# ectucker1/voxel-raytracing

Measured on AMD Instinct MI355X. Metric: Mrays/sec at 1080p treehouse.vox; achieved HBM GB/s vs MI355X peak, higher is better.
Workload: dtype f32; 1 GPU; synthetic:treehouse(seed=2) 256^3 stand-in for treehouse.vox, 1920x1080, primary rays only (BASELINE configs[1]); 128 frame(s)/step (128 per GPU, consecutive poses, one K1 launch per step), 16-row strips over 1 GPU(s); traversal=AUTO, bytes_out_per_px=37, device=AMD Radeon Graphics (gfx950:sramecc+:xnack-)

## Files before the change

voxel-raytracing_amd/csrc/vrt_api.hip:

```cpp
#include <cstdio>
#include <cstdlib>
#include <cstring>

#include "image_io.h"
#include "vox_reader.h"
#include "vrt_host.h"

using namespace vrt;

static thread_local std::string g_err;

int vrt::fail(int code, const std::string& msg) { g_err = msg; return code; }

struct OptName { const char* name; const char* env; int DevOptions::*field; };
static const OptName kOptNames[] = {
    {"tile_tags", "VRT_TILE_TAGS", &DevOptions::tile_tags}, {"box_rect", "VRT_BOX_RECT", &DevOptions::box_rect},
    {"xcd_regions", "VRT_XCD_REGIONS", &DevOptions::xcd_regions}, {"fast_loop", "VRT_FAST_LOOP", &DevOptions::fast_loop},
    {"no_bounce_kernel", "VRT_NO_BOUNCE_KERNEL", &DevOptions::no_bounce_kernel}, {"sky_fast", "VRT_SKY_FAST", &DevOptions::sky_fast},
    {"sky_span", "VRT_SKY_SPAN", &DevOptions::sky_span},
    {"packed_bounces", "VRT_PACKED_BOUNCES", &DevOptions::packed_bounces}, {"ao_batch", "VRT_AO_BATCH", &DevOptions::ao_batch}, {"tags_async", "VRT_TAGS_ASYNC", &DevOptions::tags_async},
    {"hit_table", "VRT_HIT_TABLE", &DevOptions::hit_table},
    {"thresh_runs", "VRT_THRESH_RUNS", &DevOptions::thresh_runs}, {"denoise_th16", "VRT_DENOISE_TH", &DevOptions::denoise_th16}, {"denoise_packed", "VRT_DENOISE_PACKED", &DevOptions::denoise_packed},
    {"denoise_pair", "VRT_DENOISE_PAIR", &DevOptions::denoise_pair}, {"denoise_p0", "VRT_DENOISE_P0", &DevOptions::denoise_p0}, {"denoise_pair_wgs", "VRT_DENOISE_PAIR_WGS", &DevOptions::denoise_pair_wgs},
    {"denoise_verified", "VRT_DENOISE_VERIFIED", &DevOptions::denoise_verified}, {"denoise_guard_div8", "VRT_DENOISE_GUARD_DIV8", &DevOptions::denoise_guard_div8},
    {"denoise_count", "VRT_DENOISE_COUNT", &DevOptions::denoise_count},
    {"open_cells", "VRT_OPEN_CELLS", &DevOptions::open_cells}, {"df_prefetch", "VRT_DF_PREFETCH", &DevOptions::df_prefetch},
    {"df_own", "VRT_DF_OWN", &DevOptions::df_own},
};

extern "C" {

const char* vrt_last_error(void) { return g_err.c_str(); }

int vrt_ctx_create(int device, vrt_ctx** out)
{
    if (!out) return fail(VRT_ERR_INVALID, "vrt_ctx_create: out is NULL");
    int n = 0;
    hipError_t e = hipGetDeviceCount(&n);
    if (e != hipSuccess || n <= 0)
        return fail(VRT_ERR_NO_DEVICE, std::string("no HIP device available (") + hipGetErrorString(e) +
                                           "); this library has no CPU fallback");
    if (device < 0 || device >= n) return fail(VRT_ERR_INVALID, "vrt_ctx_create: device index out of range");
    HIPCHK(hipSetDevice(device));
    vrt_ctx* c = new vrt_ctx();
    c->device = device;
    for (const OptName& o : kOptNames) {
        const char* e = getenv(o.env);
        if (e && e[0] >= '0' && e[0] <= '9') c->opt.*(o.field) = atoi(e);
    }
    if (hipStreamCreateWithFlags(&c->stream, hipStreamNonBlocking) != hipSuccess) { delete c; return fail(VRT_ERR_HIP, "hipStreamCreate failed"); }
    hipEventCreate(&c->ev_geo0); hipEventCreate(&c->ev_prim1); hipEventCreate(&c->ev_geo1);
    hipEventCreate(&c->ev_den0); hipEventCreate(&c->ev_den1);
    *out = c;
    return VRT_OK;
}

void vrt_ctx_destroy(vrt_ctx* c)
{
    if (!c) return;
    hipSetDevice(c->device);
    hipStreamSynchronize(c->stream);
    if (c->tag_stream) { hipStreamSynchronize(c->tag_stream); hipStreamDestroy(c->tag_stream); }
    for (int b = 0; b < 2; b++) {
        if (c->tag_done[b]) hipEventDestroy(c->tag_done[b]);
        if (c->tag_read[b]) hipEventDestroy(c->tag_read[b]);
    }
    if (c->upload_stream) { hipStreamSynchronize(c->upload_stream); hipStreamDestroy(c->upload_stream); }
    for (int i = 0; i < vrt_ctx::kTabRing; i++) {
        if (c->tab_host[i]) hipHostFree(c->tab_host[i]);
        if (c->tab_uploaded[i]) hipEventDestroy(c->tab_uploaded[i]);
        if (c->tab_consumed[i]) hipEventDestroy(c->tab_consumed[i]);
    }
// ... 341 lines not shown
    p.xcd_turn = (n > 1 && p.tiles_y_local > 0 && ceil_div(p.tiles_y_local, 8) * 8 * 100 > p.tiles_y_local * 103) ? 1 : 0;
    p.wgs_per_frame_rcp = p.wgs_per_frame ? (uint32_t)(0x100000000ull / (uint64_t)p.wgs_per_frame) : 0u;
    {
        const bool want = opt.xcd_regions != 0;
        if (want && n >= 8 && p.sh.nranks == 1 && p.tile_h == 8 && p.tiles_x >= 4 && p.tiles_y_local >= 8) {
            const uint32_t rw = ((uint32_t)p.tiles_x + 1u) / 2u, rh = ((uint32_t)p.tiles_y_local + 3u) / 4u;
            p.xcd_turn = 2;
            p.wgs_per_frame = rw * rh;
            p.wgs_per_frame_rcp = (uint32_t)(0x100000000ull / (uint64_t)p.wgs_per_frame);
            p.tiles_y_rcp = (uint32_t)(0x100000000ull / (uint64_t)rw);
        }
    }
    p.tps = (uint32_t)(p.sh.strip_rows / p.tile_h);
    p.tiles_x_rcp = (uint32_t)(0x100000000ull / (uint64_t)p.tiles_x);
    if (p.xcd_turn != 2) p.tiles_y_rcp = p.tiles_y_local ? (uint32_t)(0x100000000ull / (uint64_t)p.tiles_y_local) : 0u;
    p.tps_rcp = (uint32_t)(0x100000000ull / (uint64_t)p.tps);
    p.fused_shade = (st->ao_samples == 0 && st->shadows == 0 && (st->max_bounces == 0 || !s->metallic_voxels)) ? 1 : ((st->flags & VRT_FLAG_SPLIT_KERNELS) ? 0 : 2);
    p.no_bounce = ((st->max_bounces == 0 || !s->metallic_voxels) && opt.no_bounce_kernel) ? 1 : 0;
    p.sc.vol.ao_batch = (opt.ao_batch && p.sc.vol.df_own) ? 1u : 0u;
    p.packed_chain = (opt.packed_bounces && st->ao_samples <= 0xFFFFu && (!s->bricks || opt.packed_bounces >= 2)) ? 1 : 0;
    {
        const bool want = opt.fast_loop != 0;
        const bool df = st->traversal == VRT_TRAVERSAL_AUTO || st->traversal == VRT_TRAVERSAL_DF;
        const bool sec = p.fused_shade != 1;
        bool ok = want && df && s->d.vol.df_fast && st->max_steps >= 1 && st->max_steps <= 1024 && p.tile_h == 8 &&
                  !(st->flags & (VRT_FLAG_DEBUG_PLANES | 2u)) && (!sec || st->ao_samples == 0 || (st->ao_steps >= 1 && st->ao_steps <= 1024));
        for (int f = 0; f < n && ok; f++) ok = frames[f].hit_voxel == nullptr;
        p.fast_loop = ok ? ((counts || (st->flags & VRT_FLAG_MARCHED_COUNTS)) ? 2 : 1) : 0;
        if (s->bricks && (counts || (st->flags & (VRT_FLAG_MARCHED_COUNTS | VRT_FLAG_DEBUG_PLANES | 2u)))) p.fast_loop = 2;
        const int dmax = s->d.vol.W > s->d.vol.H ? (s->d.vol.W > s->d.vol.D ? s->d.vol.W : s->d.vol.D) : (s->d.vol.H > s->d.vol.D ? s->d.vol.H : s->d.vol.D);
        p.sc.vol.df_thresh = (ok && opt.thresh_runs && !counts && dmax <= 1022 && st->max_steps >= 32) ? 1u : 0u;
        if (s->bricks) p.sc.vol.df_thresh = (opt.thresh_runs && !counts && !(st->flags & (VRT_FLAG_DEBUG_PLANES | 2u)) && st->max_steps >= 32) ? 1u : 0u;
    }
    {
        bool ok = opt.sky_fast != 0 && s->d.skyk.w != 0u && !(st->flags & (VRT_FLAG_DEBUG_PLANES | 2u));
        for (int f = 0; f < n && ok; f++)
            ok = !frames[f].color_f && !frames[f].hit_voxel && !frames[f].hit_mask && !frames[f].steps_primary && !frames[f].steps_total && !frames[f].rays_total;
        p.sky_fast = ok ? 1 : 0;
    }
    p.occ2_bytes = s->occ2_bytes; p.occ3_bytes = s->occ3_bytes;
    p.occ_in_lds = ((size_t)s->occ2_bytes + s->occ3_bytes <= 65536) ? 1 : 0;
    {
        TileMap& m = p.map;
        bool six = p.sky_fast != 0;
        for (int f = 0; f < n && six; f++)
            six = frames[f].color8 && frames[f].depth && frames[f].motion && frames[f].mask8 && frames[f].position && frames[f].normal8 &&
                  !frames[f].hit_id && !frames[f].color8_strips;
        m.flags = (st->flags & 0xFFFFu) | (p.sky_fast ? VRT_MAPFLAG_SKY_FAST : 0u) | (six ? VRT_MAPFLAG_SIX : 0u) |
                  ((p.sky_fast && opt.sky_span) ? VRT_MAPFLAG_SKY_SPAN : 0u); m.n_frames = p.n_frames; m.xcd_turn = p.xcd_turn;
        m.wgs_per_frame = p.wgs_per_frame; m.wgs_per_frame_rcp = p.wgs_per_frame_rcp;
        m.tiles_x = p.tiles_x; m.tiles_x_rcp = p.tiles_x_rcp; m.tiles_y_local = p.tiles_y_local; m.tiles_y_rcp = p.tiles_y_rcp;
        m.tps = p.tps; m.tps_rcp = p.tps_rcp; m.tile = p.tile_h; m.nranks = p.sh.nranks; m.strip_rows = p.sh.strip_rows;
        m.W = p.W; m.H = p.H;
    }
    return VRT_OK;
}

static int launch_records(vrt_ctx* c, size_t px, GeomParams& p)
{
    if (c->records_px < px) {
        HIPCHK(hipStreamSynchronize(c->stream));
        c->records.reset(); c->hit_list.reset(); c->records_px = 0;
        HIPCHK(c->records.alloc(px * sizeof(uint4)));
        HIPCHK(c->hit_list.alloc((px + 1) * sizeof(uint32_t)));
        c->records_px = px;
    }
    p.records = c->records.get();
    p.hit_list = c->hit_list.get();
    p.hit_count = c->hit_list.get() + c->records_px;
    HIPCHK(hipMemsetAsync(p.hit_count, 0, sizeof(uint32_t), c->stream));
    return VRT_OK;
}

static int launch_tags(vrt_ctx* c, const vrt_scene* s, const Launch& l, const FrameSlot* slots, int tab, bool counts, GeomParams& p, int* tag_buf)
{
    const int n = l.n;
    bool want = c->opt.tile_tags != 0 && s->cells_ok && !counts && l.W <= 8128 && l.H <= 8128;
    bool any = false;
    for (int f = 0; f < n && want && !any; f++) any = !(slots[f].box[0] == 0 && slots[f].box[1] == 255 && slots[f].box[2] == 0 && slots[f].box[3] == 255);
    const bool tags = want && any;
    p.tags_x = tags ? (uint32_t)(p.tiles_x * (p.tile_w / 8)) : 0u; p.tags_y = tags ? (uint32_t)(p.tiles_y_local * (p.tile_h / 8)) : 0u;
    p.tags_per_frame = p.tags_x * p.tags_y + 1u;
    const size_t words = (size_t)p.tags_per_frame * (size_t)n;
    const int b = c->tag_flip; c->tag_flip ^= 1;
    *tag_buf = b;
    if (c->tile_tags_words[b] < words) {
        HIPCHK(hipStreamSynchronize(c->stream));
        if (c->tag_stream) HIPCHK(hipStreamSynchronize(c->tag_stream));
        c->tile_tags[b].reset(); c->tile_tags_words[b] = 0;
        HIPCHK(c->tile_tags[b].alloc(words * sizeof(uint32_t)));
        HIPCHK(hipMemsetAsync(c->tile_tags[b].get(), 0, words * sizeof(uint32_t), c->stream));
        HIPCHK(hipStreamSynchronize(c->stream));
        c->tile_tags_words[b] = words;
        c->tag_read_valid[b] = false;
    }
    if (++c->tile_gen == 0u) {
        HIPCHK(hipStreamSynchronize(c->stream));
        if (c->tag_stream) HIPCHK(hipStreamSynchronize(c->tag_stream));
        for (int q = 0; q < 2; q++)
            if (c->tile_tags[q]) HIPCHK(hipMemsetAsync(c->tile_tags[q].get(), 0, c->tile_tags_words[q] * sizeof(uint32_t), c->stream));
        HIPCHK(hipStreamSynchronize(c->stream));
        c->tile_gen = 1u;
    }
    p.tile_tags = c->tile_tags[b].get(); p.tile_gen = c->tile_gen;
    if (!tags) {
        std::vector<uint32_t> ones((size_t)n, c->tile_gen);
// ... 196 lines not shown
```

voxel-raytracing_amd/csrc/vrt_device.hip:

```cpp
#include "vrt_device_common.h"

namespace vrt {


struct RayHit {
    uint32_t material;
    f3 pos, normal, dir;
    uint32_t ncode;
};

typedef const __attribute__((address_space(3))) uint64_t* lds_u64_ptr;
template <bool LDS> struct OccT;
template <> struct OccT<true>  { lds_u64_ptr o2, o3; };
template <> struct OccT<false> { const uint64_t* o2; const uint64_t* o3; };

__device__ __forceinline__ f3 hit_normal(uint32_t mask, int sx, int sy, int sz)
{
    const uint32_t k = __builtin_popcount(mask & 7u);
    const float c = k == 1u ? 1.0f : (k == 2u ? __uint_as_float(0x3f3504f3u) : __uint_as_float(0x3f13cd3au));
    const bool general = ((mask & 1u) && sx == 0) || ((mask & 2u) && sy == 0) || ((mask & 4u) && sz == 0);
    f3 n = mk3((mask & 1u) ? (float)(-sx) : 0.0f, (mask & 2u) ? (float)(-sy) : 0.0f, (mask & 4u) ? (float)(-sz) : 0.0f);
    if (general) return normalize3(n);
    return mk3(n.x * c, n.y * c, n.z * c);
}
// ... 729 lines not shown
        }
    }
    if (MODE != 0) {
        f3 col;
        if (MODE >= 5) {
            PixCtx c; c.px = px; c.py = py; c.fetches = 0; c.rays = 0; c.pc = SlotOf<TABLE>::push(P, frame);
            c.ldsw = (uint32_t)(uintptr_t)(lds_u64_ptr)lds_occ + (uint32_t)wave * (uint32_t)VRT_AO_SLOT;
            f3 colh = mk3(0.0f, 0.0f, 0.0f);
            if (__ballot(hit) != 0ull) colh = color_main_ray_packed<TRAV, OccT<kLds>, (MODE == 5 ? 2 : (MODE == 6 ? 5 : VRT_MAX_BOUNCES))>(P, occ, c, h, hit);
            if (hit) {
                col = colh;
                if (VRT_COUNTS(TRAV) && steps_total && !(P.st.flags & 3u)) steps_total[i] = r.fetches + c.fetches;
                if (rays_total && !(P.st.flags & 3u)) rays_total[i] = 1u + c.rays;
            } else {
                col = sky_color(s, dir);
                if (VRT_COUNTS(TRAV) && steps_total && P.sc.vol.count_lookups != 0u && !(P.st.flags & 3u)) steps_total[i] = r.fetches + c.fetches;
            }
        } else if (hit) {
            PixCtx c; c.px = px; c.py = py; c.fetches = 0; c.rays = 0; c.pc = SlotOf<TABLE>::push(P, frame);
            c.ldsw = (uint32_t)(uintptr_t)(lds_u64_ptr)lds_occ + (uint32_t)wave * (uint32_t)VRT_AO_SLOT;
            if (MODE == 1) col = color_hit<TRAV, OccT<kLds>, false>(P, occ, c, h, mk3(0.0f, 0.0f, 0.0f), 0);
            else {
                col = color_main_ray<TRAV, OccT<kLds>, MODE != 4>(P, occ, c, h);
                if (VRT_COUNTS(TRAV) && steps_total && !(P.st.flags & 3u)) steps_total[i] = r.fetches + c.fetches;
                if (rays_total && !(P.st.flags & 3u)) rays_total[i] = 1u + c.rays;
            }
        } else {
            col = sky_color(s, dir);
        }
#ifdef VRT_EXP_LATE_INDEX
        {
            int pxl = px, pyl = py;
            asm volatile("" : "+v"(pxl), "+v"(pyl));
            const size_t il = (size_t)pyl * (size_t)W + (size_t)pxl;
            store_color(f, col, il, (uint32_t)il, ((uint32_t)(yp0 + (pyl - y0)) * (uint32_t)W + (uint32_t)pxl) << 2);
        }
#else
        store_color(f, col, i, i32, ((uint32_t)(yp0 + (py - y0)) * (uint32_t)W + (uint32_t)px) << 2);
#endif
#ifdef VRT_EXP_STAMPS
        if (f.motion) *gptr<vrt_f2>(f.motion, i32 << 3) = (vrt_f2){__uint_as_float((uint32_t)t_begin), __uint_as_float((uint32_t)wall_clock64())};
#endif
    } else if (hit) {
        uint32_t packed = h.material | (r.mask << 8) | ((uint32_t)(r.sx + 1) << 11) | ((uint32_t)(r.sy + 1) << 13) |
                          ((uint32_t)(r.sz + 1) << 15);
        P.records[i] = make_uint4(__float_as_uint(h.pos.x), __float_as_uint(h.pos.y), __float_as_uint(h.pos.z), packed);
        uint32_t slot = atomicAdd(P.hit_count, 1u);
        P.hit_list[slot] = (uint32_t)i;
    } else {
        store_color(f, sky_color(s, dir), i, i32, ((uint32_t)(yp0 + (py - y0)) * (uint32_t)W + (uint32_t)px) << 2);
    }
}


template <int TRAV, bool OCC_LDS>
__global__ __launch_bounds__(256) void k_shade(const GeomParams P)
{
    extern __shared__ __attribute__((aligned(16))) uint64_t lds_occ[];
    constexpr bool kLds = OCC_LDS && (TRAV == VRT_TRAVERSAL_BITMASK || TRAV == VRT_TRAVERSAL_JUMP);
    uint32_t count = *P.hit_count;
    if (blockIdx.x * 256u >= count) return;
    const OccT<kLds> occ = stage_occ<kLds>(P, lds_occ);
    uint32_t gid = blockIdx.x * 256u + threadIdx.x;
    if (gid >= count) return;
    size_t i = P.hit_list[gid];
    int W = P.W;
    int px = (int)(i % (size_t)W), py = (int)(i / (size_t)W);

    uint4 rec = P.records[i];
    RayHit h;
    h.material = rec.w & 0xFFu;
    h.dir = primary_dir(P.slot[0], px, py);
    h.pos = mk3(__uint_as_float(rec.x), __uint_as_float(rec.y), __uint_as_float(rec.z));
    uint32_t mask = (rec.w >> 8) & 7u;
    int sx = (int)((rec.w >> 11) & 3u) - 1, sy = (int)((rec.w >> 13) & 3u) - 1, sz = (int)((rec.w >> 15) & 3u) - 1;
    PixCtx c; c.px = px; c.py = py; c.fetches = 0; c.rays = 0; c.pc = &P.slot[0].pc;
    c.ldsw = (uint32_t)(uintptr_t)(lds_u64_ptr)lds_occ + (uint32_t)__builtin_amdgcn_readfirstlane((int)(threadIdx.x >> 6)) * (uint32_t)VRT_AO_SLOT;
    h.normal = hit_normal(mask, sx, sy, sz);
    {
        const bool general = (mask & 7u) == 0u || ((mask & 1u) && sx == 0) || ((mask & 2u) && sy == 0) || ((mask & 4u) && sz == 0);
        h.ncode = general ? 0xFFFFFFFFu : ((mask & 7u) | ((uint32_t)(sx < 0) << 3) | ((uint32_t)(sy < 0) << 4) | ((uint32_t)(sz < 0) << 5));
    }
    f3 col = color_main_ray<TRAV>(P, occ, c, h);
    const vrt_frame& f = P.slot[0].fr;
    if (f.color_f) { f.color_f[i * 3 + 0] = col.x; f.color_f[i * 3 + 1] = col.y; f.color_f[i * 3 + 2] = col.z; }
    if (f.color8 || f.color8_strips) {
        uchar4 c8; c8.x = unorm8(col.x); c8.y = unorm8(col.y); c8.z = unorm8(col.z); c8.w = 0;
        if (f.color8) reinterpret_cast<uchar4*>(f.color8)[i] = c8;
        if (f.color8_strips) {
            int strip = py / P.sh.strip_rows;
            int yp = (strip / P.sh.nranks) * P.sh.strip_rows + (py - strip * P.sh.strip_rows);
            reinterpret_cast<uchar4*>(f.color8_strips)[(size_t)yp * (size_t)P.W + (size_t)px] = c8;
        }
    }
    if (VRT_COUNTS(TRAV) && f.steps_total) f.steps_total[i] += c.fetches;
    if (f.rays_total) f.rays_total[i] += c.rays;
}


template <int TRAV, bool OCC_LDS, int MODE, bool TABLE>
static void launch_k1_map(const GeomParams& p, dim3 grid, dim3 block, size_t lds, hipStream_t s)
{
    if constexpr (TRAV == VRT_TRAVERSAL_DF_FAST || TRAV == VRT_TRAVERSAL_BRICK) {
        if (p.xcd_turn == 0) { hipLaunchKernelGGL((k_primary<TRAV, OCC_LDS, MODE, TABLE, 0>), grid, block, lds, s, p); return; }
        if (p.xcd_turn == 2) { hipLaunchKernelGGL((k_primary<TRAV, OCC_LDS, MODE, TABLE, 2>), grid, block, lds, s, p); return; }
    }
    hipLaunchKernelGGL((k_primary<TRAV, OCC_LDS, MODE, TABLE, -1>), grid, block, lds, s, p);
}

template <int TRAV, bool OCC_LDS, bool TABLE>
static hipError_t launch_k1(const GeomParams& p, dim3 grid, dim3 block, size_t lds, hipStream_t s)
{
    constexpr bool kProduct = TRAV == VRT_TRAVERSAL_DF_FAST || TRAV == VRT_TRAVERSAL_DF_FAST_CNT || TRAV == VRT_TRAVERSAL_BRICK || TRAV == VRT_TRAVERSAL_BRICK_CNT;
    if (p.fused_shade == 1) launch_k1_map<TRAV, OCC_LDS, 1, TABLE>(p, grid, block, lds, s);
    else if (p.fused_shade == 2) {
        if (p.no_bounce) launch_k1_map<TRAV, OCC_LDS, 4, TABLE>(p, grid, block, lds, s);
        else if (kProduct && p.packed_chain) {
            if constexpr (kProduct) {
                if (p.st.max_bounces <= 2)      launch_k1_map<TRAV, OCC_LDS, 5, TABLE>(p, grid, block, lds, s);
                else if (p.st.max_bounces <= 5) launch_k1_map<TRAV, OCC_LDS, 6, TABLE>(p, grid, block, lds, s);
                else                            launch_k1_map<TRAV, OCC_LDS, 7, TABLE>(p, grid, block, lds, s);
            }
        }
        else launch_k1_map<TRAV, OCC_LDS, 2, TABLE>(p, grid, block, lds, s);
    }
    else if constexpr (TABLE) return hipErrorInvalidValue;
    else launch_k1_map<TRAV, OCC_LDS, 0, false>(p, grid, block, lds, s);
    return hipGetLastError();
}

template <int TRAV, bool OCC_LDS>
hipError_t launch_primary_t(const GeomParams& p, hipStream_t s)
{
    dim3 grid((unsigned)p.tiles_x * 8u, (unsigned)((p.tiles_y_local + 7) / 8), (unsigned)p.n_frames);
    if (p.xcd_turn == 2) grid = dim3(8u * (((unsigned)p.tiles_x + 1u) / 2u), ((unsigned)p.tiles_y_local + 3u) / 4u, (unsigned)p.n_frames);
    else if (p.xcd_turn) grid = dim3((unsigned)p.tiles_x * 8u * (unsigned)((p.tiles_y_local * p.n_frames + 7) / 8));
    dim3 block(p.tile_h == 8 ? 64 : 256);
    size_t lds = (OCC_LDS && (TRAV == VRT_TRAVERSAL_BITMASK || TRAV == VRT_TRAVERSAL_JUMP)) ? p.occ2_bytes + p.occ3_bytes : 0;
    if ((TRAV == VRT_TRAVERSAL_DF_FAST || TRAV == VRT_TRAVERSAL_DF_FAST_CNT || TRAV == VRT_TRAVERSAL_BRICK || TRAV == VRT_TRAVERSAL_BRICK_CNT) && p.fused_shade != 1)
        lds = (size_t)(block.x / 64u) * (size_t)VRT_AO_SLOT;
    return p.table ? launch_k1<TRAV, OCC_LDS, true>(p, grid, block, lds, s) : launch_k1<TRAV, OCC_LDS, false>(p, grid, block, lds, s);
}

template <int TRAV, bool OCC_LDS>
hipError_t launch_shade_t(const GeomParams& p, hipStream_t s)
{
    dim3 grid((unsigned)(((size_t)p.total_tiles * p.tile_w * p.tile_h + 255) / 256)), block(256);
    size_t lds = (OCC_LDS && (TRAV == VRT_TRAVERSAL_BITMASK || TRAV == VRT_TRAVERSAL_JUMP)) ? p.occ2_bytes + p.occ3_bytes : 0;
    if (TRAV == VRT_TRAVERSAL_DF_FAST || TRAV == VRT_TRAVERSAL_DF_FAST_CNT || TRAV == VRT_TRAVERSAL_BRICK || TRAV == VRT_TRAVERSAL_BRICK_CNT) lds = 4u * (size_t)VRT_AO_SLOT;
    hipLaunchKernelGGL((k_shade<TRAV, OCC_LDS>), grid, block, lds, s, p);
    return hipGetLastError();
}

#define VRT_K1_K2(EXT, TRAV, OCC_LDS)                                                          \
    EXT template hipError_t launch_primary_t<TRAV, OCC_LDS>(const GeomParams&, hipStream_t);   \
    EXT template hipError_t launch_shade_t<TRAV, OCC_LDS>(const GeomParams&, hipStream_t);
#define VRT_PART_0(EXT) VRT_K1_K2(EXT, VRT_TRAVERSAL_BRICK, false)
#define VRT_PART_1(EXT) VRT_K1_K2(EXT, VRT_TRAVERSAL_DF_FAST, false)
#define VRT_PART_2(EXT) VRT_K1_K2(EXT, VRT_TRAVERSAL_DF_FAST_CNT, false) VRT_K1_K2(EXT, VRT_TRAVERSAL_BRICK_CNT, false)
#define VRT_PART_3(EXT) VRT_K1_K2(EXT, VRT_TRAVERSAL_DENSE, false) VRT_K1_K2(EXT, VRT_TRAVERSAL_DF, false) VRT_K1_K2(EXT, VRT_TRAVERSAL_DFJ, false) \
                        VRT_K1_K2(EXT, VRT_TRAVERSAL_BITMASK, false) VRT_K1_K2(EXT, VRT_TRAVERSAL_BITMASK, true)                                     \
                        VRT_K1_K2(EXT, VRT_TRAVERSAL_JUMP, false) VRT_K1_K2(EXT, VRT_TRAVERSAL_JUMP, true)
VRT_PART_0(extern) VRT_PART_1(extern) VRT_PART_2(extern) VRT_PART_3(extern)
#define VRT_PART_N(N) VRT_PART_##N
#define VRT_PART(N) VRT_PART_N(N)
VRT_PART(VRT_K1_PART)()

#if VRT_K1_PART == 0

__global__ void k_sky_normals(const DevScene s, float4* table)
{
    const uint32_t code = threadIdx.x & 63u, mask = code & 7u;
    const int sx = (code & 8u) ? -1 : 1, sy = (code & 16u) ? -1 : 1, sz = (code & 32u) ? -1 : 1;
    f3 c = mk3(0.0f, 0.0f, 0.0f);
    if (mask != 0u) c = sky_color(s, hit_normal(mask, sx, sy, sz));
    table[code] = make_float4(c.x, c.y, c.z, 0.0f);
}

hipError_t launch_sky_normals(const DevScene& sc, float* table, hipStream_t s)
{
    hipLaunchKernelGGL(k_sky_normals, dim3(1), dim3(64), 0, s, sc, reinterpret_cast<float4*>(table));
    return hipGetLastError();
}

__global__ __launch_bounds__(256) void k_sky_rgba8(const float4* __restrict__ sky, uint32_t* __restrict__ sky8, size_t n)
{
    const size_t i = (size_t)blockIdx.x * blockDim.x + threadIdx.x;
    if (i >= n) return;
    const float4 t = sky[i];
    sky8[i] = (uint32_t)unorm8(t.x) | ((uint32_t)unorm8(t.y) << 8) | ((uint32_t)unorm8(t.z) << 16);
}

hipError_t launch_sky_rgba8(const float* sky, uint32_t* sky8, size_t n, hipStream_t s)
{
    hipLaunchKernelGGL(k_sky_rgba8, dim3((unsigned)((n + 255) / 256)), dim3(256), 0, s, reinterpret_cast<const float4*>(sky), sky8, n);
    return hipGetLastError();
}

__global__ __launch_bounds__(256) void k_debug_sky(const DevScene s, const float* __restrict__ v, size_t n, uint32_t* __restrict__ out)
{
    const size_t i = (size_t)blockIdx.x * blockDim.x + threadIdx.x;
    if (i >= n) return;
    const float vx = v[3 * i], vy = v[3 * i + 1], vz = v[3 * i + 2];
    const f3 d = normalize3(mk3(vx, vy, vz));
    const float u = atan2_spec(d.z, d.x) * 0.1591f + 0.5f;
    const float w = asin_spec(-d.y) * 0.3183f + 0.5f;
    const uint32_t sx = wrap_texel(u, s.sky_w), sy = wrap_texel(w, s.sky_h);
    uint32_t tx = 0u, ty = 0u;
    float un = 0.0f, vn = 0.0f;
    const bool sure = s.skyk.w != 0u && sky_texel_fast(vx, vy, vz, s.skyk, tx, ty, un, vn);
    out[4 * i] = sx | (sy << 16); out[4 * i + 1] = tx | (ty << 16); out[4 * i + 2] = sure ? 1u : 0u; out[4 * i + 3] = __float_as_uint(un);
}

hipError_t debug_brick_counts(unsigned long long out[4])
{
// ... 154 lines not shown
```

voxel-raytracing_amd/csrc/vrt_host.h:

```cpp
#pragma once
#include <mutex>
#include <string>
#include <vector>

#include "vrt_internal.h"

namespace vrt {

int fail(int code, const std::string& msg);

#define HIPCHK(expr)                                                                              \
    do {                                                                                          \
        hipError_t e_ = (expr);                                                                   \
        if (e_ != hipSuccess)                                                                     \
            return ::vrt::fail(VRT_ERR_HIP, std::string(#expr) + ": " + hipGetErrorString(e_));   \
    } while (0)

inline int ceil_div(int a, int b) { return (a + b - 1) / b; }

template <class T>
class DevBuf {
public:
    DevBuf() = default;
    DevBuf(DevBuf&& o) noexcept : p_(o.p_), bytes_(o.bytes_) { o.p_ = nullptr; o.bytes_ = 0; }
    DevBuf& operator=(DevBuf&& o) noexcept
    {
        if (this != &o) { reset(); p_ = o.p_; bytes_ = o.bytes_; o.p_ = nullptr; o.bytes_ = 0; }
        return *this;
    }
    DevBuf(const DevBuf&) = delete;
    DevBuf& operator=(const DevBuf&) = delete;
    ~DevBuf() { reset(); }

    hipError_t alloc(size_t bytes)
    {
        reset();
        const hipError_t e = hipMalloc((void**)&p_, bytes);
        if (e != hipSuccess) p_ = nullptr; else bytes_ = bytes;
        return e;
    }
    void reset() { if (p_) hipFree(p_); p_ = nullptr; bytes_ = 0; }
    T* get() const { return p_; }
    size_t bytes() const { return bytes_; }
    explicit operator bool() const { return p_ != nullptr; }

private:
    T* p_ = nullptr;
    size_t bytes_ = 0;
};

}

struct DevOptions {
    int tile_tags = 1;
    int box_rect = 1;
    int xcd_regions = 0;
    int fast_loop = 1;
    int no_bounce_kernel = 1;
    int packed_bounces = 1;
    int tags_async = 0;
    int ao_batch = 1;
    int sky_fast = 1;
    int sky_span = 1;
    int thresh_runs = 1;
    int hit_table = 1;
    int denoise_th16 = 0;
    int denoise_packed = 1;
    int denoise_pair = 1;
    int denoise_p0 = 1;
    int denoise_pair_wgs = 0;
    int denoise_verified = 1;
    int denoise_guard_div8 = 0;
    int denoise_count = 0;
    int open_cells = 1;
    int df_prefetch = 1;
    int df_own = 1;
};

struct vrt_ctx {
    int device = 0;
    DevOptions opt;
    hipStream_t stream = nullptr;
    bool own_stream = true;
    bool timing = true;
    hipEvent_t ev_geo0 = nullptr, ev_prim1 = nullptr, ev_geo1 = nullptr, ev_den0 = nullptr, ev_den1 = nullptr;
    bool have_geo = false, have_den = false;
    vrt::DevBuf<uint4> records;
    vrt::DevBuf<uint32_t> hit_list;
    size_t records_px = 0;
    int div_w = 0, div_h = 0, div_ok = 0;
    uint64_t checked_ptrs[3] = {0, 0, 0};
    static constexpr int kTabRing = 4;
    vrt::DevBuf<vrt::FrameSlot> tab_dev[kTabRing];
    vrt::FrameSlot* tab_host[kTabRing] = {nullptr, nullptr, nullptr, nullptr};
    hipEvent_t tab_uploaded[kTabRing] = {nullptr, nullptr, nullptr, nullptr};
    hipEvent_t tab_consumed[kTabRing] = {nullptr, nullptr, nullptr, nullptr};
    bool tab_busy[kTabRing] = {false, false, false, false};
    int tab_next = 0;
    hipStream_t upload_stream = nullptr;
    vrt::DevBuf<uint32_t> tile_tags[2];
    size_t tile_tags_words[2] = {0, 0};
    uint32_t tile_gen = 0;
    int tag_flip = 0;
    hipStream_t tag_stream = nullptr;
    hipEvent_t tag_done[2] = {nullptr, nullptr};
    hipEvent_t tag_read[2] = {nullptr, nullptr};
    bool tag_read_valid[2] = {false, false};
    vrt::DevBuf<uint32_t> hit_colors;
    uint64_t hit_scene_gen = 0;
    vrt::DevBuf<uint32_t> den_counts;
    int den_last_passes = 0;
    vrt_settings hit_settings{};
};

struct vrt_scene {
    vrt::DevScene d{};
// ... 54 lines not shown
```

voxel-raytracing_amd/csrc/vrt_internal.h:

```cpp
#pragma once

#include <hip/hip_runtime.h>
#include <stdint.h>

#include "../../include/vrt.h"
#include "vrt_traverse.h"
#include "vrt_sky.h"
#include "vrt_tags.h"
#include "vrt_span.h"
#include "vrt_edit.h"
#include "vrt_brick_edit.h"
#include "vrt_reproject.h"
#include "vrt_upsample.h"

namespace vrt {

struct DevScene {
    VolumeView vol;
    const vrt_material* palette;
    const float*   sky;   uint32_t sky_w, sky_h;
    const float*   sky_normals;
    const uint8_t* noise; uint32_t noise_w, noise_h;
    const uint32_t* sky8;
    SkyFastConsts  skyk;
// ... 43 lines not shown
    auto det3 = [](const double* x, const double* y, const double* z) {
        return x[0] * (y[1] * z[2] - y[2] * z[1]) - y[0] * (x[1] * z[2] - x[2] * z[1]) + z[0] * (x[1] * y[2] - x[2] * y[1]);
    };
    const double det = det3(U, V, C);
    const double scale = (fabs(U[0]) + fabs(U[1]) + fabs(U[2])) * (fabs(V[0]) + fabs(V[1]) + fabs(V[2])) * (fabs(C[0]) + fabs(C[1]) + fabs(C[2]));
    if (!(fabs(det) > 1e-9 * scale) || !(scale > 0.0)) return;
    double x0 = 1e300, x1 = -1e300, y0 = 1e300, y1 = -1e300;
    for (int k = 0; k < 8; k++) {
        const double P[3] = {((k & 1) ? dim[0] + m : -m) - cam[0], ((k & 2) ? dim[1] + m : -m) - cam[1], ((k & 4) ? dim[2] + m : -m) - cam[2]};
        const double lam = det3(U, V, P) / det, a = det3(P, V, C) / det, b = det3(U, P, C) / det;
        const double reach = fabs(P[0]) + fabs(P[1]) + fabs(P[2]);
        if (!(lam > 1e-3 * reach / (fabs(C[0]) + fabs(C[1]) + fabs(C[2]) + 1e-30))) return;
        const double px = (a / lam + 1.0) * 0.5 * W, py = (b / lam + 1.0) * 0.5 * H;
        if (!(px == px) || !(py == py)) return;
        x0 = px < x0 ? px : x0; x1 = px > x1 ? px : x1; y0 = py < y0 ? py : y0; y1 = py > y1 ? py : y1;
    }
    const double margin = 4.0;
    auto lo = [](double v) { v = floor(v / 32.0); return v < 0.0 ? 0.0 : (v > 255.0 ? 255.0 : v); };
    auto hi = [](double v) { v = ceil(v / 32.0); return v < 0.0 ? 0.0 : (v > 255.0 ? 255.0 : v); };
    out[0] = (uint8_t)lo(x0 - margin); out[1] = (uint8_t)hi(x1 + margin);
    out[2] = (uint8_t)lo(y0 - margin); out[3] = (uint8_t)hi(y1 + margin);
}

__host__ __device__ inline float screen_div_fast(float x, float n, float r)
{
    float q = x * r;
    return __builtin_fmaf(__builtin_fmaf(-q, n, x), r, q);
}
inline bool screen_div_exact(int n)
{
    const float fn = (float)n, r = 1.0f / fn;
    for (int i = 0; i < n; i++) {
        const float x = (float)i + 0.5f;
        volatile float want = x / fn;
        if (screen_div_fast(x, fn, r) != want) return false;
    }
    return true;
}

struct FrameSlot {
    RayGenConsts rg;
    vrt_push     pc;
    vrt_frame    fr;
    int32_t      shard_rank;
    uint8_t      box[4];
};
static_assert(sizeof(FrameSlot) == 256, "FrameSlot is sized for aligned scalar loads");

#define VRT_MAX_BATCH 8
#define VRT_MAX_TABLE 256

#define VRT_MAPFLAG_SKY_FAST 0x10000u
#define VRT_MAPFLAG_SKY_SPAN 0x40000u
#define VRT_MAPFLAG_SIX      0x20000u
struct alignas(64) TileMap {
    uint32_t flags;
    int32_t  n_frames, xcd_turn;
    uint32_t wgs_per_frame, wgs_per_frame_rcp;
    int32_t  tiles_x;       uint32_t tiles_x_rcp;
    int32_t  tiles_y_local; uint32_t tiles_y_rcp;
    uint32_t tps, tps_rcp;
    int32_t  tile;
    int32_t  nranks, strip_rows;
    int32_t  W, H;
};
static_assert(sizeof(TileMap) == 64, "TileMap is one 16-dword scalar load");

struct GeomParams {
    FrameSlot  slot[VRT_MAX_BATCH];
    TileMap    map;
    const FrameSlot* table;
    int32_t    n_frames;
    int32_t    xcd_turn;
    uint32_t   wgs_per_frame, wgs_per_frame_rcp;
    int32_t    W, H;
    float      rcp_w, rcp_h;
    int32_t    fast_screen_div;
    DevScene   sc;
    vrt_settings st;
    ShardMap   sh;
    int32_t    tile_w, tile_h;
    int32_t    tiles_x, tiles_y_local, total_tiles, chunk;
    uint32_t   tiles_y_rcp;
    uint32_t   tiles_x_rcp, tps, tps_rcp;
    uint4*     records;
    uint32_t*  hit_count;
    uint32_t*  hit_list;
    int32_t    fused_shade;
    int32_t    no_bounce;
    int32_t    packed_chain;
    int32_t    fast_loop;
    int32_t    occ_in_lds;
    int32_t    sky_fast;
    uint32_t   occ2_bytes, occ3_bytes;
    uint32_t*  tile_tags;
    uint32_t   tile_gen, tags_x, tags_y, tags_per_frame;
    const uint32_t* cells;
    uint32_t   n_cells, cell_size;
    const uint32_t* hit_colors;
};

#define VRT_DENOISE_SEGS 64
struct DenoiseParams {
    const uint8_t* color_in;
    const int8_t*  normal;
    const float*   position;
// ... 131 lines not shown
```

voxel-raytracing_amd/csrc/vrt_span.h:

```cpp
#pragma once

#include "vrt_spec.h"

namespace vrt {

VRT_HD uint32_t span_x0(uint32_t col8) { return (col8 & ~3u) << 3; }
VRT_HD uint32_t span_role(uint32_t col8) { return col8 & 3u; }

VRT_HD bool span_in_frame(uint32_t x0, uint32_t W) { return x0 + 32u <= W; }

VRT_HD bool block_skips(uint32_t box, uint32_t px0, uint32_t py0, bool untagged)
{
    const uint32_t bx = px0 >> 5, by = py0 >> 5;
    return box != 0xFF00FF00u && (bx < (box & 0xFFu) || bx >= ((box >> 8) & 0xFFu) || by < ((box >> 16) & 0xFFu) || by >= (box >> 24) || untagged);
}

VRT_HD bool span_untagged(uint32_t t0, uint32_t t1, uint32_t t2, uint32_t t3, uint32_t tag_all, uint32_t tile_gen)
{
    return t0 != tile_gen && t1 != tile_gen && t2 != tile_gen && t3 != tile_gen && tag_all != tile_gen;
}

VRT_HD bool span_eligible(uint32_t t0, uint32_t t1, uint32_t t2, uint32_t t3, uint32_t tag_all, uint32_t tile_gen, uint32_t box,
                          uint32_t x0, uint32_t py0, uint32_t W)
{
    return span_in_frame(x0, W) && block_skips(box, x0, py0, span_untagged(t0, t1, t2, t3, tag_all, tile_gen));
}

VRT_HD void span_pixel(bool span, uint32_t x0, uint32_t py0, uint32_t role, uint32_t lane, int& px, int& py)
{
    const uint32_t mask = span ? 31u : 7u, sh = span ? 5u : 3u;
    px = (int)(x0 + (lane & mask));
    py = (int)(py0 + (span ? 2u * role : 0u) + (lane >> sh));
}

}
```

Baseline: 94930 Mrays/s.

## Add span-wave primary kernel covering 32-pixel spans per wave with vectorized sky stores

Adds a new primary-ray kernel in which each 64-thread wave covers a 32x8 span. Fully sky spans are written with four-pixel-per-lane vector nontemporal stores of the zero planes and the sky color. Other spans loop over four 8x8 blocks, reloading kernel arguments per block to keep register pressure low. It is gated by a new default-on option that requires batches larger than the max slot batch plus several other flags, and the kernel is only compiled in a new part 4. The tile mapping switches to span columns, so it risks load imbalance and depends on build configuration.

```diff
diff --git a/voxel-raytracing_amd/csrc/vrt_api.hip b/voxel-raytracing_amd/csrc/vrt_api.hip
--- a/voxel-raytracing_amd/csrc/vrt_api.hip
+++ b/voxel-raytracing_amd/csrc/vrt_api.hip
@@ -17,7 +17,7 @@
     {"tile_tags", "VRT_TILE_TAGS", &DevOptions::tile_tags}, {"box_rect", "VRT_BOX_RECT", &DevOptions::box_rect},
     {"xcd_regions", "VRT_XCD_REGIONS", &DevOptions::xcd_regions}, {"fast_loop", "VRT_FAST_LOOP", &DevOptions::fast_loop},
     {"no_bounce_kernel", "VRT_NO_BOUNCE_KERNEL", &DevOptions::no_bounce_kernel}, {"sky_fast", "VRT_SKY_FAST", &DevOptions::sky_fast},
-    {"sky_span", "VRT_SKY_SPAN", &DevOptions::sky_span},
+    {"sky_span", "VRT_SKY_SPAN", &DevOptions::sky_span}, {"span_waves", "VRT_SPAN_WAVES", &DevOptions::span_waves},
     {"packed_bounces", "VRT_PACKED_BOUNCES", &DevOptions::packed_bounces}, {"ao_batch", "VRT_AO_BATCH", &DevOptions::ao_batch}, {"tags_async", "VRT_TAGS_ASYNC", &DevOptions::tags_async},
     {"hit_table", "VRT_HIT_TABLE", &DevOptions::hit_table},
     {"thresh_runs", "VRT_THRESH_RUNS", &DevOptions::thresh_runs}, {"denoise_th16", "VRT_DENOISE_TH", &DevOptions::denoise_th16}, {"denoise_packed", "VRT_DENOISE_PACKED", &DevOptions::denoise_packed},
@@ -465,6 +465,14 @@
         m.tiles_x = p.tiles_x; m.tiles_x_rcp = p.tiles_x_rcp; m.tiles_y_local = p.tiles_y_local; m.tiles_y_rcp = p.tiles_y_rcp;
         m.tps = p.tps; m.tps_rcp = p.tps_rcp; m.tile = p.tile_h; m.nranks = p.sh.nranks; m.strip_rows = p.sh.strip_rows;
         m.W = p.W; m.H = p.H;
+#ifndef VRT_EXP_STAMPS
+        if ((opt.span_waves >= 2 || (opt.span_waves == 1 && n > VRT_MAX_BATCH)) && (m.flags & VRT_MAPFLAG_SKY_SPAN) && six && p.fused_shade == 1 && opt.hit_table && p.fast_loop == 1 && !s->bricks &&
+            p.tile_h == 8) {
+            m.flags |= VRT_MAPFLAG_SPAN_WAVES;
+            m.tiles_x = ceil_div(W, 32);
+            m.tiles_x_rcp = (uint32_t)(0x100000000ull / (uint64_t)m.tiles_x);
+        }
+#endif
     }
     return VRT_OK;
 }
diff --git a/voxel-raytracing_amd/csrc/vrt_device.hip b/voxel-raytracing_amd/csrc/vrt_device.hip
--- a/voxel-raytracing_amd/csrc/vrt_device.hip
+++ b/voxel-raytracing_amd/csrc/vrt_device.hip
@@ -805,6 +805,245 @@
     }
 }
 
+#if VRT_K1_PART == 4
+typedef float    vrt_f4u __attribute__((ext_vector_type(4), aligned(4)));
+typedef uint32_t vrt_u4u __attribute__((ext_vector_type(4), aligned(4)));
+typedef uint32_t vrt_u1b __attribute__((aligned(1)));
+
+typedef const __attribute__((address_space(4))) char* const_byte_ptr;
+template <bool TABLE> struct SpanArgs {
+    const_byte_ptr ka, sl;
+    static __device__ __forceinline__ SpanArgs make(const FrameSlot* table, uint32_t frame)
+    {
+        SpanArgs a;
+        a.ka = (const_byte_ptr)__builtin_amdgcn_kernarg_segment_ptr();
+        asm volatile("" : "+s"(a.ka));
+        a.sl = TABLE ? (const_byte_ptr)(table + frame) : a.ka + offsetof(GeomParams, slot) + (size_t)frame * sizeof(FrameSlot);
+        asm volatile("" : "+s"(a.sl));
+        return a;
+    }
+    template <int N> static __device__ __forceinline__ void words(const_byte_ptr p, size_t off, void* dst)
+    {
+        const_u32_ptr w = (const_u32_ptr)(p + off);
+        uint32_t tmp[N];
+#pragma unroll
+        for (int i = 0; i < N; i++) tmp[i] = w[i];
+        __builtin_memcpy(dst, tmp, sizeof tmp);
+    }
+    __device__ __forceinline__ void sky(SkyFastConsts& k, const uint32_t*& sky8) const
+    {
+        static_assert(offsetof(DevScene, skyk) == offsetof(DevScene, sky8) + 8 && sizeof(SkyFastConsts) == 40, "sky8 and skyk are read as one block");
+        uint32_t tmp[12];
+        words<12>(ka, offsetof(GeomParams, sc) + offsetof(DevScene, sky8), tmp);
+        __builtin_memcpy(&sky8, tmp, 8);
+        __builtin_memcpy(&k, tmp + 2, sizeof k);
+    }
+    __device__ __forceinline__ void raygen(RayGenConsts& g, float& crx, float& cry, float& crz, float& rcp_w, float& rcp_h, int& fast_div) const
+    {
+        static_assert(offsetof(GeomParams, rcp_h) == offsetof(GeomParams, rcp_w) + 4 && offsetof(GeomParams, fast_screen_div) == offsetof(GeomParams, rcp_w) + 8, "rcp_w, rcp_h, fast_screen_div are read as one block");
+        float cr[3]; uint32_t q[3];
+        words<sizeof(RayGenConsts) / 4>(sl, offsetof(FrameSlot, rg), &g);
+        words<3>(sl, offsetof(FrameSlot, pc) + offsetof(vrt_push, cam_right), cr);
+        words<3>(ka, offsetof(GeomParams, rcp_w), q);
+        crx = cr[0]; cry = cr[1]; crz = cr[2];
+        rcp_w = __uint_as_float(q[0]); rcp_h = __uint_as_float(q[1]); fast_div = (int)q[2];
+    }
+    __device__ __forceinline__ f3 cam_pos() const
+    {
+        float c[3];
+        words<3>(sl, offsetof(FrameSlot, pc) + offsetof(vrt_push, cam_pos), c);
+        return mk3(c[0], c[1], c[2]);
+    }
+    __device__ __forceinline__ void planes(void** out) const
+    {
+        static_assert(offsetof(vrt_frame, color8) == 0 && offsetof(vrt_frame, depth) == 8 && offsetof(vrt_frame, motion) == 16 && offsetof(vrt_frame, mask8) == 24 &&
+                      offsetof(vrt_frame, position) == 32 && offsetof(vrt_frame, normal8) == 40, "vrt_frame layout");
+        words<12>(sl, offsetof(FrameSlot, fr), out);
+    }
+    __device__ __forceinline__ void scene(GeomParams& L) const
+    {
+        words<sizeof(DevScene) / 4>(ka, offsetof(GeomParams, sc), &L.sc);
+        words<sizeof(vrt_settings) / 4>(ka, offsetof(GeomParams, st), &L.st);
+        words<2>(ka, offsetof(GeomParams, hit_colors), &L.hit_colors);
+    }
+};
+
+template <bool TABLE, int MAP>
+__global__ __launch_bounds__(64) __attribute__((amdgpu_waves_per_eu(8, 8))) void k_primary_span(const GeomParams P)
+{
+    TileMap M = P.map;
+    int ty, tx;
+    uint32_t frame;
+    if (!block_to_tile<MAP>(M, frame, ty, tx)) return;
+    const uint32_t tile_gen = P.tile_gen;
+    uint32_t st0, st1, st2, st3, tag_all;
+    {
+        const_u32_ptr tg = (const_u32_ptr)(P.tile_tags + (size_t)frame * P.tags_per_frame);
+        const uint32_t tags_x = P.tags_x, row = (uint32_t)ty * tags_x;
+        st0 = tg[row + span_tag_col((uint32_t)tx, 0u, tags_x)]; st1 = tg[row + span_tag_col((uint32_t)tx, 1u, tags_x)];
+        st2 = tg[row + span_tag_col((uint32_t)tx, 2u, tags_x)]; st3 = tg[row + span_tag_col((uint32_t)tx, 3u, tags_x)];
+        tag_all = tg[P.tags_per_frame - 1u];
+    }
+    RayGenConsts g;
+    float cam_right[3];
+    int shard_rank;
+    uint32_t box;
+    SlotOf<TABLE>::head(P, frame, g, cam_right, shard_rank, box);
+    asm volatile("" : "+s"(box));
+    float crx = cam_right[0], cry = cam_right[1], crz = cam_right[2];
+    float rcp_w = P.rcp_w, rcp_h = P.rcp_h;
+    int fast_div = P.fast_screen_div;
+    asm volatile("" : "+s"(g.cd.x), "+s"(g.cd.y), "+s"(g.cd.z), "+s"(g.planeV.x), "+s"(g.planeV.y), "+s"(g.planeV.z), "+s"(g.jx), "+s"(g.jy),
+                      "+s"(g.W), "+s"(g.H), "+s"(crx), "+s"(cry), "+s"(crz), "+s"(shard_rank),
+                      "+s"(rcp_w), "+s"(rcp_h), "+s"(fast_div), "+s"(st0), "+s"(st1), "+s"(st2), "+s"(st3), "+s"(tag_all));
+    int xt, y0, yp0;
+    if (!tile_origin(M, ty, tx, shard_rank, xt, y0, yp0)) return;
+    const uint32_t x0 = (uint32_t)tx << 5;
+    const int W = M.W, H = M.H;
+    const uint32_t lane = threadIdx.x;
+    const uint32_t tagged = (uint32_t)__builtin_amdgcn_readfirstlane((int)(((st0 == tile_gen) ? 1u : 0u) | ((st1 == tile_gen) ? 2u : 0u) | ((st2 == tile_gen) ? 4u : 0u) |
+                                                                           ((st3 == tile_gen) ? 8u : 0u) | ((tag_all == tile_gen) ? 15u : 0u)));
+    const bool whole = span_eligible(st0, st1, st2, st3, tag_all, tile_gen, box, x0, (uint32_t)y0, (uint32_t)W);
+
+    if (whole) {
+        SkyFastConsts k;
+        const uint32_t* sky8;
+        const SpanArgs<TABLE> A = SpanArgs<TABLE>::make(P.table, frame);
+        A.sky(k, sky8);
+        void* pl[6];
+        A.planes(pl);
+        int px, py;
+        span_quad(x0, (uint32_t)y0, lane, px, py);
+        const bool in = py < H;
+        uint32_t sx[4], sy[4];
+        bool sure = true;
+#pragma unroll
+        for (int j = 0; j < 4; j++) {
+            const f3 v = primary_v(g, crx, cry, crz, rcp_w, rcp_h, fast_div, px + j, py);
+            sure = sky_texel_fast(v.x, v.y, v.z, k, sx[j], sy[j]) & sure;
+        }
+        if (__ballot(in && !sure) == 0ull) {
+            if (!in) return;
+            vrt_u4u c8;
+            c8.x = *gptr<const uint32_t>(sky8, (sy[0] * k.w + sx[0]) << 2); c8.y = *gptr<const uint32_t>(sky8, (sy[1] * k.w + sx[1]) << 2);
+            c8.z = *gptr<const uint32_t>(sky8, (sy[2] * k.w + sx[2]) << 2); c8.w = *gptr<const uint32_t>(sky8, (sy[3] * k.w + sx[3]) << 2);
+            const uint32_t row = (uint32_t)py * (uint32_t)W + x0;
+            const vrt_f4u zf = {0.0f, 0.0f, 0.0f, 0.0f};
+            const vrt_u4u zu = {0u, 0u, 0u, 0u};
+#pragma unroll
+            for (uint32_t q = 0; q < 4u; q++) __builtin_nontemporal_store(zf, gptr<vrt_f4u>(pl[4], (row << 4) + span_zero_chunk(lane, q)));
+#pragma unroll
+            for (uint32_t q = 0; q < 2u; q++) __builtin_nontemporal_store(zf, gptr<vrt_f4u>(pl[2], (row << 3) + span_zero_chunk(lane, q)));
+            __builtin_nontemporal_store(zf, gptr<vrt_f4u>(pl[1], (row << 2) + span_zero_chunk(lane, 0u)));
+            __builtin_nontemporal_store(zu, gptr<vrt_u4u>(pl[5], (row << 2) + span_zero_chunk(lane, 0u)));
+            __builtin_nontemporal_store((vrt_u1b)0u, gptr<vrt_u1b>(pl[3], row + ((lane & 7u) << 2)));
+            *gptr<vrt_u4u>(pl[0], ((uint32_t)py * (uint32_t)W + (uint32_t)px) << 2) = c8;
+            return;
+        }
+    }
+
+    const uint32_t nblk = span_blocks(x0, (uint32_t)W);
+    for (uint32_t kb = 0; kb < nblk; kb++) {
+        const SpanArgs<TABLE> A = SpanArgs<TABLE>::make(P.table, frame);
+        GeomParams Q;
+        A.scene(Q);
+        uint32_t ln = lane, bxw = box;
+        float zf = 0.0f;
+        asm volatile("" : "+v"(ln), "+s"(bxw), "+v"(zf));
+        const DevScene& s = Q.sc;
+        const OccT<false> occ = stage_occ<false>(Q, nullptr);
+        int px, py;
+        span_block_pixel(x0, (uint32_t)y0, kb, ln, px, py);
+        if (px >= W || py >= H) continue;
+        const uint32_t i32 = (uint32_t)py * (uint32_t)W + (uint32_t)px;
+        f3 v;
+        {
+            RayGenConsts gb;
+            float bx, by, bz, rw, rh;
+            int fd;
+            A.raygen(gb, bx, by, bz, rw, rh, fd);
+            v = primary_v(gb, bx, by, bz, rw, rh, fd, px, py);
+        }
+        const bool skip = block_skips(bxw, x0 + 8u * kb, (uint32_t)y0, ((tagged >> kb) & 1u) == 0u);
+        f3 start = mk3(0.0f, 0.0f, 0.0f), dir;
+        RayHit h; RayInt r;
+        if (skip) {
+            SkyFastConsts k;
+            const uint32_t* sky8;
+            A.sky(k, sky8);
+            uint32_t sx, sy;
+            const bool sure = sky_texel_fast(v.x, v.y, v.z, k, sx, sy);
+            if (__ballot(!sure) == 0ull) {
+                const uint32_t c8 = *gptr<const uint32_t>(sky8, (sy * k.w + sx) << 2);
+                void* pl[6];
+                A.planes(pl);
+                *gptr<vrt_f4>(pl[4], i32 << 4) = (vrt_f4){zf, zf, zf, zf};
+                *gptr<vrt_f2>(pl[2], i32 << 3) = (vrt_f2){zf, zf};
+                *gptr<float>(pl[1], i32 << 2) = zf;
+                *gptr<uint32_t>(pl[5], i32 << 2) = 0u;
+                *gptr<uint8_t>(pl[3], i32) = (uint8_t)0;
+                *gptr<uint32_t>(pl[0], i32 << 2) = c8;
+                continue;
+            }
+            dir = primary_normalize(v);
+            h.material = 0u; h.dir = dir; h.pos = mk3(0.0f, 0.0f, 0.0f); h.normal = mk3(0.0f, 0.0f, 0.0f); h.ncode = 0xFFFFFFFFu;
+        } else {
+            asm volatile("" :: "s"(Q.sc.vol.W), "s"(Q.sc.vol.H), "s"(Q.sc.vol.D), "s"(Q.st.max_steps), "s"(Q.sc.vol.df), "s"(Q.sc.vol.df_stride),
+                               "s"(Q.sc.vol.vox));
+            start = A.cam_pos();
+            dir = primary_normalize(v);
+            trace_ray<VRT_TRAVERSAL_DF_FAST, OccT<false>, true>(s, occ, start, dir, Q.st.max_steps, h, r);
+        }
+        const bool hit = h.material != 0;
+        void* pl[6];
+        A.planes(pl);
+        float depth = 0.0f;
+        if (hit) depth = len3(mk3(h.pos.x - start.x, h.pos.y - start.y, h.pos.z - start.z));
+        uint32_t n = 0u;
+        if (hit) n = (uint32_t)(uint8_t)snorm8(h.normal.x) | ((uint32_t)(uint8_t)snorm8(h.normal.y) << 8) | ((uint32_t)(uint8_t)snorm8(h.normal.z) << 16);
+        *gptr<float>(pl[1], i32 << 2) = depth;
+        *gptr<vrt_f2>(pl[2], i32 << 3) = (vrt_f2){zf, zf};
+        *gptr<uint8_t>(pl[3], i32) = hit ? (uint8_t)230 : (uint8_t)0;
+        *gptr<vrt_f4>(pl[4], i32 << 4) = (vrt_f4){h.pos.x, h.pos.y, h.pos.z, 0.0f};
+        *gptr<uint32_t>(pl[5], i32 << 2) = n;
+        uint32_t c8;
+        if (__ballot(hit && h.ncode == 0xFFFFFFFFu) == 0ull) {
+            if (hit) c8 = *gptr<const uint32_t>(Q.hit_colors, ((h.material << 6) | h.ncode) << 2);
+            else {
+                const f3 col = sky_color(s, dir);
+                c8 = (uint32_t)unorm8(col.x) | ((uint32_t)unorm8(col.y) << 8) | ((uint32_t)unorm8(col.z) << 16);
+            }
+        } else {
+            f3 col;
+            if (hit) {
+                PixCtx c; c.px = px; c.py = py; c.fetches = 0; c.rays = 0; c.pc = SlotOf<TABLE>::push(P, frame); c.ldsw = 0u;
+                col = color_hit<VRT_TRAVERSAL_DF_FAST, OccT<false>, false>(Q, occ, c, h, mk3(0.0f, 0.0f, 0.0f), 0);
+            } else col = sky_color(s, dir);
+            c8 = (uint32_t)unorm8(col.x) | ((uint32_t)unorm8(col.y) << 8) | ((uint32_t)unorm8(col.z) << 16);
+        }
+        *gptr<uint32_t>(pl[0], i32 << 2) = c8;
+    }
+}
+
+template <bool TABLE>
+static void launch_span_map(const GeomParams& p, dim3 grid, hipStream_t s)
+{
+    if (p.xcd_turn == 0)      hipLaunchKernelGGL((k_primary_span<TABLE, 0>), grid, dim3(64), 0, s, p);
+    else if (p.xcd_turn == 2) hipLaunchKernelGGL((k_primary_span<TABLE, 2>), grid, dim3(64), 0, s, p);
+    else                      hipLaunchKernelGGL((k_primary_span<TABLE, -1>), grid, dim3(64), 0, s, p);
+}
+
+hipError_t launch_primary_span(const GeomParams& p, hipStream_t s)
+{
+    const unsigned sx = (unsigned)p.map.tiles_x;
+    dim3 grid(sx * 8u, (unsigned)((p.tiles_y_local + 7) / 8), (unsigned)p.n_frames);
+    if (p.xcd_turn == 2) grid = dim3(8u * ((sx + 1u) / 2u), ((unsigned)p.tiles_y_local + 3u) / 4u, (unsigned)p.n_frames);
+    else if (p.xcd_turn) grid = dim3(sx * 8u * (unsigned)((p.tiles_y_local * p.n_frames + 7) / 8));
+    if (p.table) launch_span_map<true>(p, grid, s); else launch_span_map<false>(p, grid, s);
+    return hipGetLastError();
+}
+#endif
+
 
 template <int TRAV, bool OCC_LDS>
 __global__ __launch_bounds__(256) void k_shade(const GeomParams P)
@@ -882,9 +1121,14 @@
     return hipGetLastError();
 }
 
+hipError_t launch_primary_span(const GeomParams& p, hipStream_t s);
+
 template <int TRAV, bool OCC_LDS>
 hipError_t launch_primary_t(const GeomParams& p, hipStream_t s)
 {
+#if VRT_K1_PART == 1
+    if constexpr (TRAV == VRT_TRAVERSAL_DF_FAST && !OCC_LDS) { if (p.map.flags & VRT_MAPFLAG_SPAN_WAVES) return launch_primary_span(p, s); }
+#endif
     dim3 grid((unsigned)p.tiles_x * 8u, (unsigned)((p.tiles_y_local + 7) / 8), (unsigned)p.n_frames);
     if (p.xcd_turn == 2) grid = dim3(8u * (((unsigned)p.tiles_x + 1u) / 2u), ((unsigned)p.tiles_y_local + 3u) / 4u, (unsigned)p.n_frames);
     else if (p.xcd_turn) grid = dim3((unsigned)p.tiles_x * 8u * (unsigned)((p.tiles_y_local * p.n_frames + 7) / 8));
@@ -914,6 +1158,7 @@
 #define VRT_PART_3(EXT) VRT_K1_K2(EXT, VRT_TRAVERSAL_DENSE, false) VRT_K1_K2(EXT, VRT_TRAVERSAL_DF, false) VRT_K1_K2(EXT, VRT_TRAVERSAL_DFJ, false) \
                         VRT_K1_K2(EXT, VRT_TRAVERSAL_BITMASK, false) VRT_K1_K2(EXT, VRT_TRAVERSAL_BITMASK, true)                                     \
                         VRT_K1_K2(EXT, VRT_TRAVERSAL_JUMP, false) VRT_K1_K2(EXT, VRT_TRAVERSAL_JUMP, true)
+#define VRT_PART_4(EXT)
 VRT_PART_0(extern) VRT_PART_1(extern) VRT_PART_2(extern) VRT_PART_3(extern)
 #define VRT_PART_N(N) VRT_PART_##N
 #define VRT_PART(N) VRT_PART_N(N)
diff --git a/voxel-raytracing_amd/csrc/vrt_host.h b/voxel-raytracing_amd/csrc/vrt_host.h
--- a/voxel-raytracing_amd/csrc/vrt_host.h
+++ b/voxel-raytracing_amd/csrc/vrt_host.h
@@ -62,6 +62,7 @@
     int ao_batch = 1;
     int sky_fast = 1;
     int sky_span = 1;
+    int span_waves = 1;
     int thresh_runs = 1;
     int hit_table = 1;
     int denoise_th16 = 0;
diff --git a/voxel-raytracing_amd/csrc/vrt_internal.h b/voxel-raytracing_amd/csrc/vrt_internal.h
--- a/voxel-raytracing_amd/csrc/vrt_internal.h
+++ b/voxel-raytracing_amd/csrc/vrt_internal.h
@@ -119,6 +119,7 @@
 
 #define VRT_MAPFLAG_SKY_FAST 0x10000u
 #define VRT_MAPFLAG_SKY_SPAN 0x40000u
+#define VRT_MAPFLAG_SPAN_WAVES 0x80000u
 #define VRT_MAPFLAG_SIX      0x20000u
 struct alignas(64) TileMap {
     uint32_t flags;
diff --git a/voxel-raytracing_amd/csrc/vrt_span.h b/voxel-raytracing_amd/csrc/vrt_span.h
--- a/voxel-raytracing_amd/csrc/vrt_span.h
+++ b/voxel-raytracing_amd/csrc/vrt_span.h
@@ -33,4 +33,26 @@
     py = (int)(py0 + (span ? 2u * role : 0u) + (lane >> sh));
 }
 
+
+VRT_HD uint32_t span_count(uint32_t W) { return (W + 31u) >> 5; }
+VRT_HD uint32_t span_blocks(uint32_t x0, uint32_t W) { const uint32_t n = (W - x0 + 7u) >> 3; return n < 4u ? n : 4u; }
+
+VRT_HD uint32_t span_tag_col(uint32_t span, uint32_t k, uint32_t tags_x)
+{
+    const uint32_t c = 4u * span + k;
+    return tags_x == 0u ? 0u : (c < tags_x ? c : tags_x - 1u);
 }
+
+VRT_HD void span_quad(uint32_t x0, uint32_t py0, uint32_t lane, int& px, int& py)
+{
+    px = (int)(x0 + 4u * (lane & 7u));
+    py = (int)(py0 + (lane >> 3));
+}
+VRT_HD void span_block_pixel(uint32_t x0, uint32_t py0, uint32_t k, uint32_t lane, int& px, int& py)
+{
+    px = (int)(x0 + 8u * k + (lane & 7u));
+    py = (int)(py0 + (lane >> 3));
+}
+VRT_HD uint32_t span_zero_chunk(uint32_t lane, uint32_t q) { return ((q << 3) + (lane & 7u)) << 4; }
+
+}
```

After: 93950 Mrays/s. -1.0%, worse.
